# liznerski/eoe

Hardware: AMD Instinct MI355X
Metric: train images/sec, CLIP ViT-B/32 + HSC, 224x224 (higher is better)
Workload: dtype fp16; 1 GPU; CLIP ViT-B/32 (12 layers) + Linear(512,256) + HSC, full fine-tune, Adam lr 1e-4 wd 1e-3, 224x224, 128 normal + 128 OE images per GPU per step; global_batch=256, parallelism=dp1, launch=eager, weight-gradient launches on a side stream under the dgrad chain, arithmetic=16-bit MFMA operands, fp32 accumulate

## Files before the change

### eoe_amd/_lib.py

```python
import ctypes as C
import os
import re

import torch

from . import _build

ABI_VERSION = 5
EOE_F16, EOE_BF16, EOE_F32 = 1, 2, 3
EOE_RESIZE_BILINEAR, EOE_RESIZE_BICUBIC = 2, 3
EOE_MSM_LPF, EOE_MSM_HPF, EOE_MSM_BLUR = 1, 2, 3
EOE_MSM_FORM_NONE, EOE_MSM_FORM_DENSE, EOE_MSM_FORM_RANK = 0, 1, 2
EOE_GCN_L1, EOE_GCN_L2 = 1, 2
EOE_SALIENCY_MAX, EOE_SALIENCY_L2, EOE_SALIENCY_GRADXINPUT = 0, 1, 2
EOE_FUSE_MEAN, EOE_FUSE_MAX, EOE_FUSE_MIN = 0, 1, 2
EOE_CAM_GRADCAM, EOE_CAM_HIRESCAM = 0, 1
EOE_COMM_I64, EOE_COMM_ID_BYTES, EOE_COMM_ALGO_RING, EOE_COMM_ALGO_RS_AG = 8, 128, 0, 1
EPI_NONE, EPI_GELU, EPI_RESIDUAL, EPI_GELU_BWD = 0, 1, 2, 3
NT_KERNELS = ("none", "persistent_256x128", "persistent_256x96", "narrow_256x64", "persistent_narrow", "two_wg_128", "two_wg_160",
              "wide_160x256x32", "one_wave_160x256", "one_wave_256x256", "eight_wave", "eight_wave_stream_k", "split_k", "gather")
(NT_KERNEL_NONE, NT_KERNEL_PERSISTENT_256x128, NT_KERNEL_PERSISTENT_256x96, NT_KERNEL_NARROW_256x64, NT_KERNEL_PERSISTENT_NARROW,
 NT_KERNEL_TWO_WG_128, NT_KERNEL_TWO_WG_160, NT_KERNEL_WIDE_160x256x32, NT_KERNEL_ONE_WAVE_160x256, NT_KERNEL_ONE_WAVE_256x256,
 NT_KERNEL_EIGHT_WAVE, NT_KERNEL_EIGHT_WAVE_STREAM_K, NT_KERNEL_SPLIT_K, NT_KERNEL_GATHER) = range(14)
ADAM_CHUNK, ADAM_GROUPS = 8192, 4
# ... 100 lines not shown


class VitBlockBwdArgs(C.Structure):
    _fields_ = [("f", VitBlockFwdArgs), ("dx_out", _vp), ("dx_in", _vp),
                ("g_ln1_g", _vp), ("g_ln1_b", _vp), ("g_ln2_g", _vp), ("g_ln2_b", _vp),
                ("g_b_in", _vp), ("g_b_out", _vp), ("g_b_fc", _vp), ("g_b_proj", _vp),
                ("g_w_in", _vp), ("g_w_out", _vp), ("g_w_fc", _vp), ("g_w_proj", _vp),
                ("accumulate", _i32),
                ("d16_a", _vp), ("d16_b", _vp), ("d16_c", _vp), ("dh", _vp), ("dqkv", _vp), ("dx_mid", _vp), ("red_scratch", _vp),
                ("tn_workspace", _vp), ("tn_workspace_bytes", _i64),
                ("next_d16", _vp), ("in_d16", _vp), ("in_red_scratch", _vp), ("async_wgrad", _i32), ("red_table", C.POINTER(RedTable))]


ALLREDUCE_FN = C.CFUNCTYPE(C.c_int, C.c_void_p, C.c_void_p, C.c_int64, C.c_int, C.c_void_p)

SIGNATURES = {
    "eoe_abi_version": [],
    "eoe_struct_size": [C.c_int],
    "eoe_last_error": [],
    "eoe_vit_side_join": [_vp],
    "eoe_red_table_flush": [C.POINTER(RedTable), _vp],
    "eoe_gemm_nt": [C.POINTER(GemmArgs), _vp],
    "eoe_gemm_nt_route": [C.POINTER(GemmArgs), C.c_int, C.POINTER(C.c_int)],
    "eoe_gemm_tn": [C.POINTER(GemmArgs), _vp],
    "eoe_gemm_tn_grouped": [C.POINTER(GemmArgs), C.c_int, _vp],
    "eoe_cast_transpose": [_vp, _vp, _vp, C.c_int, C.c_int, C.c_int, _vp],
    "eoe_cast_transpose_multi": [_vp, C.c_int, C.c_int, _vp],
    "eoe_conv_pack_weight_multi": [_vp, C.c_int, C.c_int, _vp],
    "eoe_patchify": [_vp, _vp, _vp, _vp, C.c_int, C.c_int, C.c_int, C.c_int, _vp],
    "eoe_embed_lnpre_fwd": [_vp] * 8 + [C.c_int, C.c_int, C.c_int, _f32, _vp],
    "eoe_embed_lnpre_bwd": [_vp] * 10 + [C.c_int, C.c_int, C.c_int, C.c_int, _vp],
    "eoe_layernorm_fwd": [_vp, C.c_int, _vp, _vp, _vp, _vp, C.c_int, C.c_int, _f32, C.c_int, C.c_int, _vp],
    "eoe_layernorm_bwd": [_vp, C.c_int, _vp, C.c_int, _vp, _vp, _vp, _vp, C.c_int, _vp, _vp, _vp, _vp, _vp, C.c_int,
                          C.c_int, C.c_int, _vp],
    "eoe_linear_small_fwd": [_vp, _vp, _vp, _vp, C.c_int, C.c_int, C.c_int, _vp],
    "eoe_linear_small_bwd": [_vp, _vp, _vp, _vp, _vp, _vp, C.c_int, C.c_int, C.c_int, C.c_int, _vp],
    "eoe_zero_multi": [C.POINTER(_vp), C.POINTER(C.c_int), C.c_int, _vp],
    "eoe_cast_colsum": [_vp, _vp, _vp, _vp, C.c_int, C.c_int, C.c_int, C.c_int, _vp],
    "eoe_colsum": [_vp, C.c_int, _vp, C.c_int, C.c_int, C.c_int, C.c_int, _vp],
    "eoe_colsum_det": [_vp, C.c_int, _vp, _vp, C.c_int, C.c_int, C.c_int, _vp],
    "eoe_cast": [_vp, _vp, _sz, C.c_int, _vp],
    "eoe_attn_fwd": [_vp, _vp, C.c_int, C.c_int, C.c_int, C.c_int, _vp],
    "eoe_attn_bwd": [_vp, _vp, _vp, _vp, _vp, C.c_int, C.c_int, C.c_int, C.c_int, _vp],
    "eoe_attn_long_fwd": [_vp, _vp, C.c_int, C.c_int, C.c_int, C.c_int, _vp],
    "eoe_attn_long_bwd": [_vp, _vp, _vp, _vp, _vp, C.c_int, C.c_int, C.c_int, C.c_int, _vp],
    "eoe_attn_causal_fwd": [_vp, _vp, C.c_int, C.c_int, C.c_int, C.c_int, _vp],
# ... 167 lines not shown
            raise ImportError(f"eoe_amd: {cls.__name__} is {C.sizeof(cls)} bytes here but {lib.eoe_struct_size(idx)} in libeoe_hip.so "
                              "(the ctypes mirror and include/eoe_hip.h disagree)")
    return lib


def get_option(name: str) -> int:
    v = C.c_int(0)
    check(lib.eoe_get_option(name.encode(), C.byref(v)), "eoe_get_option")
    return v.value


def set_option(name: str, value: int) -> int:
    old = get_option(name)
    check(lib.eoe_set_option(name.encode(), int(value)), "eoe_set_option")
    return old


def gemm_nt_route(args: GemmArgs, ncu: int = 0) -> int:
    v = C.c_int(0)
    check(lib.eoe_gemm_nt_route(C.byref(args), int(ncu), C.byref(v)), "eoe_gemm_nt_route")
    return v.value


lib = _load()


class EoeError(RuntimeError):
    pass


def check(rc: int, what: str = ""):
    if rc != 0:
        msg = lib.eoe_last_error()
        raise EoeError(f"{what}: error {rc}: {msg.decode() if msg else ''}")


def prof_enable(on: bool):
    check(lib.eoe_prof_enable(1 if on else 0), "eoe_prof_enable")


def prof_collect():
    buf = (ProfEntry * 64)()
    n = C.c_int(0)
    check(lib.eoe_prof_collect(buf, 64, C.byref(n)), "eoe_prof_collect")
    return {buf[i].name.decode(): dict(launches=buf[i].launches, total_ms=buf[i].total_ms, flops=buf[i].flops,
                                       bytes=buf[i].bytes) for i in range(n.value)}
# ... 4 lines not shown
```

### eoe_amd/csrc/gemm.hip

```cpp
#include "gemm_common.h"
#include <stdlib.h>

unsigned long long* g_stamp_buf = nullptr;
extern int g_tn_flags;
extern int g_vit_side_stream;
extern int g_attn_flags;
extern int g_tn256_launches;
int g_nt_last_kernel = EOE_NT_KERNEL_NONE;
int g_nt_last_form = 0;
extern int g_parity_flags;
template <typename T> int eoe_launch_nt256(const void* gemm_p, int epi, int mi, hipStream_t s);
bool eoe_w8_applies(const void* gemm_p, int epi);
int eoe_w8_sk_rounds(const void* gemm_p, int flags, int ncu);
template <typename T> int eoe_launch_w8(const void* gemm_p, int epi, int sk_rounds, hipStream_t s);

namespace {


template <typename T, int EPI, int NI, int FLAGS, int GATHER = 0>
__global__ __launch_bounds__(512, 2) void gemm_nt_kernel(GemmP p) {
    extern __shared__ __attribute__((aligned(16))) char smem[];
    const int tid = threadIdx.x, lane = tid & 63, wave = tid >> 6;
    constexpr int BNI = 32 * NI;
    const int tiles_n = (p.N + BNI - 1) / BNI;
    const int total_tiles = tiles_n * ((p.M + BM - 1) / BM);
    const int G = gridDim.x;
    const int my_tiles = (total_tiles - (int)blockIdx.x + G - 1) / G;
    const int nk = p.K / BK;
// ... 732 lines not shown
    int split_s = 0;
    int sk_rounds = -1;
};

int nt128_rows_mi(const GemmP& p, int ncu, bool tie_to_160) {
    const int slots = 2 * ncu;
    const long t4 = (long)cdiv(p.M, 128) * cdiv(p.N, 128), t5 = (long)cdiv(p.M, 160) * cdiv(p.N, 128);
    const long c4 = (t4 + slots - 1) / slots * 128, c5 = (t5 + slots - 1) / slots * 160;
    return (c5 < c4 || (tie_to_160 && c5 == c4)) ? 5 : 4;
}

int nt_split_s(const GemmP& p, int epi, int flags, int ncu) {
    const int nk = p.K / BK;
    if ((flags & 8192) || !p.split_k || p.M > 1024 || nk < 24 || (epi != EOE_EPI_NONE && epi != EOE_EPI_RESIDUAL) || p.colsum || p.colsum_sq || p.accumulate ||
        (p.N & 15) || (p.ldc & 3) || (epi == EOE_EPI_RESIDUAL && (p.ldaux & 3)))
        return 0;
    int S = 8;
    while (S > 1 && (nk % S) != 0) S >>= 1;
    if (S < 2 || nk / S < 3) return 0;
    if (!p.sk_part || (size_t)S * p.M * p.N > (size_t)2 * ncu * 65536) return 0;
    return S;
}

NtRoute nt_route(const GemmP& p, int epi, int gather, int flags, int ncu) {
    if (epi == EOE_EPI_NONE && p.N <= 64 && (gather == 0 || gather == 1 || gather == 2) && !(flags & 64)) {
        return {gather ? EOE_NT_KERNEL_GATHER : EOE_NT_KERNEL_NARROW_256x64};
    }
    if (gather == 1 && epi == EOE_EPI_NONE && p.N >= 128 && !(flags & 2048)) {
        return {EOE_NT_KERNEL_GATHER, p.colsum_sq ? 4 : nt128_rows_mi(p, ncu, false)};
    }
    if (gather || (epi == EOE_EPI_NONE && p.N <= 64))
        return {gather ? EOE_NT_KERNEL_GATHER : EOE_NT_KERNEL_PERSISTENT_NARROW, 0, p.N <= 64 ? 2 : 4};
    if ((flags & (128 | 256)) && epilogue_direct_ok(p, epi))
        return (flags & 256) ? NtRoute{EOE_NT_KERNEL_ONE_WAVE_256x256, 8} : NtRoute{EOE_NT_KERNEL_ONE_WAVE_160x256, 5};
    const bool big = p.K >= 4096 && p.N >= 2048;
    if (const int S = nt_split_s(p, epi, flags, ncu)) return {EOE_NT_KERNEL_SPLIT_K, 4, 0, S};
    if (!(flags & (131072 | 4 | 8 | 512)) && p.M >= 2048 && eoe_w8_applies(&p, epi)) {
        const long tiles = (long)cdiv(p.M, 256) * (p.N / 256);
        const int sk_rounds = eoe_w8_sk_rounds(&p, flags, ncu);
        if (sk_rounds >= 0) return {EOE_NT_KERNEL_EIGHT_WAVE_STREAM_K, 0, 0, 0, sk_rounds};
        if ((flags & 262144) || tiles * 100 >= ((tiles + ncu - 1) / ncu) * ncu * 85) return {EOE_NT_KERNEL_EIGHT_WAVE};
    }
    if (!(flags & (4096 | 4 | 8 | 512)) && !p.colsum_sq && (p.N % 256) == 0 && p.N >= 2048 && (p.K % 32) == 0 && p.M >= 2048) {
        const long tiles = (long)cdiv(p.M, 160) * (p.N / 256), slots = 2L * ncu;
        if (tiles * 10 >= ((tiles + slots - 1) / slots) * slots * 9) return {EOE_NT_KERNEL_WIDE_160x256x32};
    }
    const bool gelu_wide = epi == EOE_EPI_GELU && p.N >= 2048 && p.K <= 1024 && !(flags & 1024);
    if (((flags & 512) || gelu_wide) && !(flags & (4 | 8)) && epilogue_direct_ok(p, epi) && p.M >= 2048 && p.N >= 512) {
        const int nk = p.K / BK;
        long best = 0;
        int mi_best = 5;
        for (int mi : {5, 8}) {
            const long tiles = (long)cdiv(p.M, 32 * mi) * cdiv(p.N, 256);
            const long cost = ((tiles + ncu - 1) / ncu) * ((long)mi * (nk + 2) + 30);
            if (!best || cost < best) { best = cost; mi_best = mi; }
        }
        return {mi_best == 8 ? EOE_NT_KERNEL_ONE_WAVE_256x256 : EOE_NT_KERNEL_ONE_WAVE_160x256, mi_best};
    }
    if (big && !(flags & (4 | 8)) && epilogue_direct_ok(p, epi) && p.M >= 2048) return {EOE_NT_KERNEL_ONE_WAVE_256x256, 8};
    if (!p.colsum_sq && ((flags & 8) || (!big && !(flags & 4)))) {
        const bool five = (flags & 32) || (!(flags & 16) && nt128_rows_mi(p, ncu, true) == 5);
        return five ? NtRoute{EOE_NT_KERNEL_TWO_WG_160, 5} : NtRoute{EOE_NT_KERNEL_TWO_WG_128, 4};
    }
    const int t4 = cdiv(p.M, BM) * cdiv(p.N, 128), t3 = cdiv(p.M, BM) * cdiv(p.N, 96);
    const int c4 = cdiv(t4, ncu) * 4, c3 = cdiv(t3, ncu) * 3;
    const int force = (flags >> 4) & 7;
    const bool use3 = force ? (force == 3) : (c3 * 10 <= c4 * 9);
    return use3 ? NtRoute{EOE_NT_KERNEL_PERSISTENT_256x96, 0, 3} : NtRoute{EOE_NT_KERNEL_PERSISTENT_256x128, 0, 4};
}

template <typename T>
int launch_nt(const GemmP& p, int epi, int gather, hipStream_t s) {
    const int flags = g_nt_flags, ncu = num_cus();
    const NtRoute r = nt_route(p, epi, gather, flags, ncu);
    g_nt_last_kernel = r.kernel;
    g_nt_last_form = r.mi * 16 + r.ni;
    switch (r.kernel) {
        case EOE_NT_KERNEL_NARROW_256x64:
        case EOE_NT_KERNEL_GATHER:
            if (!r.mi && !r.ni) return gather == 2 ? launch_nt64<T, 2>(p, s) : (gather ? launch_nt64<T, 1>(p, s) : launch_nt64<T, 0>(p, s));
            if (r.mi) return r.mi == 5 ? launch_nt128_gather<T, 5>(p, s) : launch_nt128_gather<T, 4>(p, s);
            if (gather == 2) return r.ni == 2 ? launch_nt_conv<T, 2, 2>(p, ncu, s) : launch_nt_conv<T, 4, 2>(p, ncu, s);
            if (gather == 3) return r.ni == 2 ? launch_nt_conv<T, 2, 3>(p, ncu, s) : launch_nt_conv<T, 4, 3>(p, ncu, s);
            return r.ni == 2 ? launch_nt_conv<T, 2, 1>(p, ncu, s) : launch_nt_conv<T, 4, 1>(p, ncu, s);
        case EOE_NT_KERNEL_PERSISTENT_NARROW: return launch_nt_conv<T, 2, 0>(p, ncu, s);
        case EOE_NT_KERNEL_ONE_WAVE_160x256:
        case EOE_NT_KERNEL_ONE_WAVE_256x256: return eoe_launch_nt256<T>(&p, epi, r.mi, s);
        case EOE_NT_KERNEL_SPLIT_K: return launch_nt128_splitk<T>(p, epi, r.split_s, s);
        case EOE_NT_KERNEL_EIGHT_WAVE:
        case EOE_NT_KERNEL_EIGHT_WAVE_STREAM_K: return eoe_launch_w8<T>(&p, epi, r.sk_rounds, s);
        case EOE_NT_KERNEL_WIDE_160x256x32: return launch_nt128w<T>(p, epi, s);
        case EOE_NT_KERNEL_TWO_WG_160: return launch_nt128<T, 5>(p, epi, s);
        case EOE_NT_KERNEL_TWO_WG_128: return launch_nt128<T, 4>(p, epi, s);
        case EOE_NT_KERNEL_PERSISTENT_256x96: return launch_nt_ni<T, 3>(p, epi, flags, ncu, s);
        default: return launch_nt_ni<T, 4>(p, epi, flags, ncu, s);
    }
}
// ... 67 lines not shown
        EOE_CHECK_ARG(a->workspace && a->workspace_bytes >= 2 * (int64_t)EOE_NT_COLSUM_WORKSPACE_BYTES(a->M, a->N),
                      "gemm_nt: colstats needs a workspace of 2 * EOE_NT_COLSUM_WORKSPACE_BYTES(M, N)");
        EOE_CHECK_ARG((a->N & 15) == 0 && (a->ldc & 7) == 0 && (a->ldaux & 7) == 0 && (((uintptr_t)a->C) & 15) == 0,
                      "gemm_nt: colstats needs N %% 16 == 0 and 16-byte aligned rows of C");
        p.colsum_part = (float*)a->workspace;
        p.colsum_sq = 1;
        p.colsum_blocked = 0;
    }
    return 0;
}

void attach_stamps(GemmP& p) {
    static const int stampon = getenv("EOE_GEMM_STAMP") ? atoi(getenv("EOE_GEMM_STAMP")) : 0;
    if (stampon) {
        static unsigned long long* buf = [] { void* b = nullptr; (void)hipMalloc(&b, 4096 * 16 * 8); return (unsigned long long*)b; }();
        (void)hipMemsetAsync(buf, 0, 4096 * 16 * 8, 0);
        p.stamp = buf;
        g_stamp_buf = buf;
    }
}

}

extern "C" int eoe_gemm_nt(const eoe_gemm_args* a, void* stream) {
    GemmP p;
    int mode;
    EOE_TRY(fill_params(a, num_cus(), p, mode));
    attach_stamps(p);
    const int osz = a->out_f32 ? 4 : 2;
    static const bool by_shape = getenv("EOE_PROF_SHAPES") != nullptr;
    char pname[32] = "gemm_nt";
    if (by_shape) snprintf(pname, sizeof(pname), "nt_%dx%dx%d_e%d%s", a->M, a->N, a->K, a->epilogue, a->colsum ? "c" : "");
    ProfScope ps(pname, 2.0 * a->M * a->N * a->K,
                 2.0 * ((a->gather ? (double)a->geo.n * a->geo.H * a->geo.W * a->geo.C : (double)a->M * a->K) + (double)a->N * a->K) +
                     (double)osz * a->M * a->N *
                     (a->epilogue == EOE_EPI_GELU ? 2 : 1) + (a->epilogue == EOE_EPI_RESIDUAL ? 4.0 * a->M * a->N : 0.0) +
                     (a->epilogue == EOE_EPI_GELU_BWD ? 2.0 * a->M * a->N : 0.0), stream);
    return a->dtype == EOE_F16 ? launch_nt<f16_t>(p, a->epilogue, mode, (hipStream_t)stream)
                               : launch_nt<bf16_t>(p, a->epilogue, mode, (hipStream_t)stream);
}

extern "C" int eoe_gemm_nt_route(const eoe_gemm_args* a, int ncu, int* kernel) {
    EOE_CHECK_ARG(kernel != nullptr, "eoe_gemm_nt_route: null pointer");
    if (ncu <= 0) ncu = num_cus();
    GemmP p;
    int mode;
    EOE_TRY(fill_params(a, ncu, p, mode));
    *kernel = nt_route(p, a->epilogue, mode, g_nt_flags, ncu).kernel;
    return 0;
}

extern "C" int eoe_debug_gemm_stamps(unsigned long long* out, int n_words) {
    if (!g_stamp_buf || !out) return eoe_set_error(EOE_ERR_ARG, "gemm stamps are not enabled (EOE_GEMM_STAMP=1)");
    if (hipDeviceSynchronize() != hipSuccess) return eoe_set_error(EOE_ERR_LAUNCH, "sync failed");
    if (hipMemcpy(out, g_stamp_buf, (size_t)n_words * 8, hipMemcpyDeviceToHost) != hipSuccess)
        return eoe_set_error(EOE_ERR_LAUNCH, "copy failed");
    return 0;
}

extern "C" int eoe_set_option(const char* name, int value) {
    if (name && !strcmp(name, "nt_flags")) { g_nt_flags = value; return 0; }
    if (name && !strcmp(name, "tn_flags")) { g_tn_flags = value; return 0; }
    if (name && !strcmp(name, "vit_side_stream")) { g_vit_side_stream = value; return 0; }
    if (name && !strcmp(name, "attn_flags")) { g_attn_flags = value; return 0; }
    if (name && !strcmp(name, "parity_flags")) { g_parity_flags = value; return 0; }
    return eoe_set_error(EOE_ERR_ARG, "unknown option");
}

extern "C" int eoe_get_option(const char* name, int* value) {
    EOE_CHECK_ARG(name && value, "eoe_get_option: null pointer");
    if (!strcmp(name, "nt_flags")) { *value = g_nt_flags; return 0; }
    if (!strcmp(name, "tn_flags")) { *value = g_tn_flags; return 0; }
    if (!strcmp(name, "vit_side_stream")) { *value = g_vit_side_stream; return 0; }
    if (!strcmp(name, "attn_flags")) { *value = g_attn_flags; return 0; }
    if (!strcmp(name, "tn256_launches")) { *value = g_tn256_launches; return 0; }
    if (!strcmp(name, "nt_last_kernel")) { *value = g_nt_last_kernel; return 0; }
    if (!strcmp(name, "nt_last_form")) { *value = g_nt_last_form; return 0; }
    if (!strcmp(name, "parity_flags")) { *value = g_parity_flags; return 0; }
    return eoe_set_error(EOE_ERR_ARG, "unknown option");
}
```

### eoe_amd/csrc/vit.cpp

```cpp
#include "common.h"
#include <mutex>
#include <stdlib.h>

#define TRY(expr)                   \
    do {                            \
        int rc__ = (expr);          \
        if (rc__ != 0) return rc__; \
    } while (0)

extern int g_tn_flags;
bool eoe_tn_streamk_would_run(const eoe_gemm_args* args, int count, void* stream);
int eoe_red_table_append(eoe_red_table* t, EoeRedJobs* jobs, void* stream);
int g_vit_side_stream = 1;

namespace {

struct SideStream {
    hipStream_t s = nullptr;
    hipEvent_t fork = nullptr, join = nullptr, wgrad_done[2] = {nullptr, nullptr};
    bool ok = false;
    unsigned seq = 0;
    bool recorded[2] = {false, false};
};
SideStream* side_stream(hipStream_t main) {
    static SideStream per_dev[16];
    static std::mutex mu;
    std::lock_guard<std::mutex> lk(mu);
    int dev = 0;
    if (hipGetDevice(&dev) != hipSuccess || dev < 0 || dev >= 16) return nullptr;
    SideStream& ss = per_dev[dev];
    hipStreamCaptureStatus st = hipStreamCaptureStatusNone;
    if (hipStreamIsCapturing(main, &st) != hipSuccess || st != hipStreamCaptureStatusNone) return nullptr;
    if (!ss.ok) {
        int lo = 0, hi = 0;
        (void)hipDeviceGetStreamPriorityRange(&lo, &hi);
        if (hipStreamCreateWithPriority(&ss.s, hipStreamNonBlocking, lo) != hipSuccess) return nullptr;
        if (hipEventCreateWithFlags(&ss.fork, hipEventDisableTiming) != hipSuccess ||
            hipEventCreateWithFlags(&ss.join, hipEventDisableTiming) != hipSuccess ||
            hipEventCreateWithFlags(&ss.wgrad_done[0], hipEventDisableTiming) != hipSuccess ||
            hipEventCreateWithFlags(&ss.wgrad_done[1], hipEventDisableTiming) != hipSuccess)
            return nullptr;
        ss.ok = true;
    }
    return &ss;
}

eoe_gemm_args gemm(const void* A, const void* B, void* C, const float* bias, int M, int N, int K, int lda, int ldb,
                   int ldc, int dtype) {
    eoe_gemm_args g = {};
    g.A = A; g.B = B; g.C = C; g.bias = bias; g.aux = nullptr; g.aux_out = nullptr; g.colsum = nullptr;
    g.M = M; g.N = N; g.K = K; g.lda = lda; g.ldb = ldb; g.ldc = ldc; g.ldaux = 0;
    g.dtype = dtype; g.epilogue = EOE_EPI_NONE; g.out_f32 = 0; g.accumulate = 0; g.alpha = 1.0f;
    return g;
}
eoe_gemm_args gemm(const eoe_vit_block_fwd_args* a, const void* A, const void* B, void* C, const float* bias, int M, int N, int K, int lda,
                   int ldb, int ldc, int dtype) {
    eoe_gemm_args g = gemm(A, B, C, bias, M, N, K, lda, ldb, ldc, dtype);
    g.sk_workspace = a->nt_sk_workspace; g.sk_workspace_bytes = a->nt_sk_workspace ? a->nt_sk_workspace_bytes : 0;
    return g;
}

int check_fwd(const eoe_vit_block_fwd_args* a) {
    if (!a) return eoe_set_error(EOE_ERR_ARG, "vit_block: null args");
    if (a->n <= 0 || a->L <= 0 || a->L > EOE_ATTN_LONG_MAX_L || a->heads <= 0 || a->D != a->heads * 64)
        return eoe_set_error(EOE_ERR_ARG, "vit_block: unsupported shape n=%d L=%d D=%d heads=%d (need D = 64*heads, L <= %d)",
                             a->n, a->L, a->D, a->heads, EOE_ATTN_LONG_MAX_L);
    if (!a->ln1_g || !a->ln1_b || !a->ln2_g || !a->ln2_b || !a->b_in || !a->b_out || !a->b_fc || !a->b_proj || !a->w_in ||
        !a->w_out || !a->w_fc || !a->w_proj || !a->x_in || !a->x_mid || !a->x_out || !a->xn1 || !a->qkv || !a->att ||
        !a->xn2 || !a->hact || !a->stats1 || !a->stats2)
        return eoe_set_error(EOE_ERR_ARG, "vit_block: null pointer in arguments");
    return 0;
}

}

extern "C" int eoe_vit_block_fwd(const eoe_vit_block_fwd_args* a, void* stream) {
    TRY(check_fwd(a));
    const int M = a->n * a->L, D = a->D, H = 4 * a->D, dt = a->dtype;
    TRY(eoe_layernorm_fwd(a->x_in, D, a->ln1_g, a->ln1_b, a->xn1, a->stats1, M, D, a->eps, dt, 0, stream));
    eoe_gemm_args g = gemm(a, a->xn1, a->w_in, a->qkv, a->b_in, M, 3 * D, D, D, D, 3 * D, dt);
    TRY(eoe_gemm_nt(&g, stream));
    TRY(a->L <= 64 ? eoe_attn_fwd(a->qkv, a->att, a->n, a->L, a->heads, dt, stream)
                   : eoe_attn_long_fwd(a->qkv, a->att, a->n, a->L, a->heads, dt, stream));
    const int Mo = a->cls_only ? a->n : M, ldrow = a->cls_only ? a->L * D : D;
    g = gemm(a, a->att, a->w_out, a->x_mid, a->b_out, Mo, D, D, ldrow, D, D, dt);
    g.epilogue = EOE_EPI_RESIDUAL; g.aux = a->x_in; g.ldaux = ldrow; g.out_f32 = 1;
    TRY(eoe_gemm_nt(&g, stream));
    TRY(eoe_layernorm_fwd(a->x_mid, D, a->ln2_g, a->ln2_b, a->xn2, a->stats2, Mo, D, a->eps, dt, 0, stream));
    g = gemm(a, a->xn2, a->w_fc, a->hact, a->b_fc, Mo, H, D, D, D, H, dt);
    g.epilogue = EOE_EPI_GELU; g.aux_out = a->hpre;
    TRY(eoe_gemm_nt(&g, stream));
    g = gemm(a, a->hact, a->w_proj, a->x_out, a->b_proj, Mo, D, H, H, H, D, dt);
    g.epilogue = EOE_EPI_RESIDUAL; g.aux = a->x_mid; g.ldaux = D; g.out_f32 = 1;
    g.split_k = a->cls_only ? 1 : 0;
    TRY(eoe_gemm_nt(&g, stream));
    return 0;
}

extern "C" int eoe_vit_block_bwd(const eoe_vit_block_bwd_args* b, void* stream) {
    if (!b) return eoe_set_error(EOE_ERR_ARG, "vit_block_bwd: null args");
    const eoe_vit_block_fwd_args* a = &b->f;
    TRY(check_fwd(a));
    if (!a->hpre || !a->w_in_t || !a->w_out_t || !a->w_fc_t || !a->w_proj_t || !b->dx_out || !b->dx_in || !b->g_ln1_g || !b->g_ln1_b ||
        !b->g_ln2_g || !b->g_ln2_b || !b->g_b_in || !b->g_b_out || !b->g_b_fc || !b->g_b_proj || !b->g_w_in || !b->g_w_out ||
        !b->g_w_fc || !b->g_w_proj || !b->d16_a || !b->d16_b || !b->d16_c || !b->dh || !b->dqkv || !b->dx_mid)
        return eoe_set_error(EOE_ERR_ARG, "vit_block_bwd: null pointer in arguments");
    const int M = a->n * a->L, D = a->D, H = 4 * a->D, dt = a->dtype, acc = b->accumulate;
    hipStream_t s = (hipStream_t)stream;
    const bool cls = a->cls_only != 0;
    const int Mo = cls ? a->n : M, ldrow = cls ? a->L * D : D;
    if (cls && a->L < 4) return eoe_set_error(EOE_ERR_ARG, "vit_block_bwd: cls_only needs L >= 4");
    if (!acc && !b->red_scratch) {
        float* zp[8] = {b->g_ln1_g, b->g_ln1_b, b->g_ln2_g, b->g_ln2_b, b->g_b_fc, b->g_b_out, b->g_b_proj, b->g_b_in};
        const int zn[8] = {D, D, D, D, H, D, D, 3 * D};
        TRY(eoe_zero_multi(zp, zn, 8, stream));
    }
    EoeRedJobs jobs;
    jobs.count = 0; jobs.tile_start[0] = 0; jobs.overwrite = acc ? 0 : 1;
    struct DeferGuard {
        explicit DeferGuard(EoeRedJobs* j) { eoe_tls_defer = j; }
        ~DeferGuard() { eoe_tls_defer = nullptr; }
    } guard(b->red_scratch ? &jobs : nullptr);
    float* red_fc = b->red_scratch;
    float* red_ln2 = red_fc ? red_fc + (size_t)((M + 63) / 64) * H : nullptr;
    float* red_attn = red_fc ? red_ln2 + EOE_LN_SCRATCH(D) : nullptr;
// ... 110 lines not shown
```

### eoe_amd/models/clip_vit.py

```python
import math
from collections import OrderedDict

import torch
from torch import nn

from .. import ops


def is_causal_mask(m) -> bool:
    if not isinstance(m, torch.Tensor) or m.dim() != 2 or m.shape[0] != m.shape[1] or not m.is_floating_point():
        return False
    want = torch.full(m.shape, float("-inf"), dtype=m.dtype, device=m.device).triu_(1)
    return bool(torch.equal(m, want))


class _PackedAttention(nn.Module):

    def __init__(self, d_model: int, n_head: int):
        super().__init__()
        self.embed_dim, self.num_heads = d_model, n_head
        self.in_proj_weight = nn.Parameter(torch.empty(3 * d_model, d_model))
        self.in_proj_bias = nn.Parameter(torch.empty(3 * d_model))
        self.out_proj = nn.Linear(d_model, d_model)
        self._reset_parameters()
# ... 81 lines not shown

    def set_normalize(self, mean, std):
        if mean is None:
            self.normalize = None
        else:
            dev = self.proj.device
            self.normalize = (torch.as_tensor(mean, dtype=torch.float32, device=dev).contiguous(),
                              torch.as_tensor(std, dtype=torch.float32, device=dev).contiguous())

    def embed(self, x: torch.Tensor) -> torch.Tensor:
        if not x.is_cuda:
            raise RuntimeError("eoe_amd.VisualTransformer runs on the GPU only (no CPU fallback)")
        mean, std = self.normalize if self.normalize is not None else (None, None)
        ops.shadow.refresh([w for blk in self.transformer.resblocks
                            for w in (blk.attn.in_proj_weight, blk.attn.out_proj.weight, blk.mlp.c_fc.weight, blk.mlp.c_proj.weight)]
                           + [self.proj])
        return ops.VitEmbedFunction.apply(x, self.conv1.weight, self.class_embedding, self.positional_embedding,
                                          self.ln_pre.weight, self.ln_pre.bias, self.patch_size, mean, std)

    def forward(self, x: torch.Tensor) -> torch.Tensor:
        n = x.shape[0]
        tok = self.embed(x)
        blocks = list(self.transformer.resblocks)
        for i, blk in enumerate(blocks):
            tok = blk.forward_tokens(tok, n, cls_only=ops.VIT_CLS_ONLY_LAST and i == len(blocks) - 1)
        return ops.VitHeadFunction.apply(tok, n, self.ln_post.weight, self.ln_post.bias, self.proj)


def convert_weights(model: nn.Module) -> nn.Module:
    def mark(p):
        if p is None:
            return
        with torch.no_grad():
            p.copy_(p.to(torch.float16).to(torch.float32))
        p._eoe_fp16_weight = True

    for m in model.modules():
        if isinstance(m, (nn.Conv1d, nn.Conv2d, nn.Linear)):
            mark(m.weight)
            mark(m.bias)
        if isinstance(m, (_PackedAttention, nn.MultiheadAttention)):
            for name in ("in_proj_weight", "q_proj_weight", "k_proj_weight", "v_proj_weight", "in_proj_bias", "bias_k", "bias_v"):
                mark(getattr(m, name, None))
        for name in ("text_projection", "proj"):
            attr = getattr(m, name, None)
            if isinstance(attr, nn.Parameter):
                mark(attr)
    return model
# ... 1 lines not shown
```

### eoe_amd/ops.py

```python
import ctypes as C
import math
import os
import weakref
from collections import namedtuple
from typing import NamedTuple, Optional

import torch

from . import _lib
from ._lib import lib, check, GemmArgs, EPI_NONE, EPI_GELU, EPI_RESIDUAL, EPI_GELU_BWD

_compute_dtype = torch.float16


def set_compute_dtype(dt):
    global _compute_dtype
    if isinstance(dt, str):
        dt = {"bf16": torch.bfloat16, "bfloat16": torch.bfloat16, "fp16": torch.float16, "f16": torch.float16,
              "float16": torch.float16}[dt]
    if dt not in (torch.bfloat16, torch.float16):
        raise ValueError(f"unsupported compute dtype {dt}")
    _compute_dtype = dt


# ... 486 lines not shown
        self.seq = 0
        if self.table.count:
            check(lib.eoe_red_table_flush(C.byref(self.table), self.stream), "eoe_red_table_flush")


_vit_sweeps = {}


def _vit_live_sweeps():
    task = torch._C._current_graph_task_id()
    return [sw for sw in _vit_sweeps.values() if sw.task == task]


def vit_flush_finish():
    for sw in _vit_live_sweeps():
        sw.flush()


def vit_side_join():
    vit_flush_finish()
    check(lib.eoe_vit_side_join(_stream()), "eoe_vit_side_join")
    for sw in _vit_live_sweeps():
        sw.pending = None


VIT_CLS_ONLY_LAST = os.environ.get("EOE_VIT_CLS_ONLY", "1") != "0"


class VitBlockFunction(torch.autograd.Function):

    @staticmethod
    def forward(ctx, x, n, heads, ln1_g, ln1_b, w_in, b_in, w_out, b_out, ln2_g, ln2_b, w_fc, b_fc, w_proj, b_proj, cls_only=False):
        _chk(x)
        x = x.contiguous()
        M, D = x.shape
        L = M // n
        ws, ptr = _block_ws(M, D, x.device, _compute_dtype)
        cls_only = bool(cls_only) and L >= 4
        x_out = x.new_empty((n, D)) if cls_only else torch.empty_like(x)
        need_t = torch.is_grad_enabled()
        sh = {k: shadow.get(w, True, True) for k, w in (("in", w_in), ("out", w_out), ("fc", w_fc), ("proj", w_proj))}
        sk_ws = nt_sk_workspace(x.device)
        code = dtype_code(_compute_dtype)
        sig = (n, L, D, heads, code, _p(ln1_g), _p(ln1_b), _p(ln2_g), _p(ln2_b), _p(b_in), _p(b_out), _p(b_fc), _p(b_proj),
               _p(sh["in"][0]), _p(sh["out"][0]), _p(sh["fc"][0]), _p(sh["proj"][0]), _p(sh["in"][1]), _p(sh["out"][1]), _p(sh["fc"][1]),
               _p(sh["proj"][1]), _p(sk_ws))
# ... 2 lines not shown
            a = _lib.VitBlockFwdArgs.from_buffer_copy(hit[1])
        else:
            a = _lib.VitBlockFwdArgs()
            a.n, a.L, a.D, a.heads, a.dtype, a.eps = n, L, D, heads, code, 1e-5
            a.ln1_g, a.ln1_b, a.ln2_g, a.ln2_b = _p(ln1_g), _p(ln1_b), _p(ln2_g), _p(ln2_b)
            a.b_in, a.b_out, a.b_fc, a.b_proj = _p(b_in), _p(b_out), _p(b_fc), _p(b_proj)
            a.w_in, a.w_out, a.w_fc, a.w_proj = (_p(sh[k][0]) for k in ("in", "out", "fc", "proj"))
            a.w_in_t, a.w_out_t, a.w_fc_t, a.w_proj_t = (_p(sh[k][1]) for k in ("in", "out", "fc", "proj"))
            a.nt_sk_workspace, a.nt_sk_workspace_bytes = _p(sk_ws), sk_ws.numel()
            if len(_vit_args_cache) > 256:
                _vit_args_cache.clear()
            _vit_args_cache[id(w_in)] = (sig, bytes(a))
        a.x_in, a.x_mid, a.x_out = _p(x), ptr["x_mid"], _p(x_out)
        a.xn1, a.qkv, a.att, a.xn2, a.hpre, a.hact = (ptr[k] for k in ("xn1", "qkv", "att", "xn2", "hpre", "hact"))
        a.stats1, a.stats2 = ptr["stats1"], ptr["stats2"]
        a.cls_only = 1 if cls_only else 0
        sw = _vit_sweeps.get((x.device.index, _stream()))
        if sw is not None and sw.table.count and sw.task != torch._C._current_graph_task_id():
            sw.table.count = 0
        keep = any(ctx.needs_input_grad)
        if not keep:
            a.hpre = None
        check(lib.eoe_vit_block_fwd(C.byref(a), _stream()), "eoe_vit_block_fwd")
        ctx.save_for_backward(x, ws, ln1_g, ln1_b, w_in, b_in, w_out, b_out, ln2_g, ln2_b, w_fc, b_fc, w_proj, b_proj)
        ctx.args = a
        ctx.shadows = sh
        ctx.sk_ws = sk_ws
        return x_out

    @staticmethod
    def backward(ctx, dx_out):
        saved = ctx.saved_tensors
        x, ws = saved[0], saved[1]
        params = dict(zip(_BLOCK_PARAMS, saved[2:]))
        M, D = x.shape
        dev = x.device
        dt = torch.float16 if ctx.args.dtype == _lib.EOE_F16 else torch.bfloat16
        dx_out = dx_out.contiguous()
        dx_in = torch.empty_like(x)
        grads = {k: _grad_target(p) for k, p in params.items()}
        b = _lib.VitBlockBwdArgs()
        b.f = ctx.args
        b.dx_out, b.dx_in = _p(dx_out), _p(dx_in)
        b.g_ln1_g, b.g_ln1_b, b.g_ln2_g, b.g_ln2_b = (_p(grads[k]) for k in ("ln1_g", "ln1_b", "ln2_g", "ln2_b"))
        b.g_b_in, b.g_b_out, b.g_b_fc, b.g_b_proj = (_p(grads[k]) for k in ("b_in", "b_out", "b_fc", "b_proj"))
        b.g_w_in, b.g_w_out, b.g_w_fc, b.g_w_proj = (_p(grads[k]) for k in ("w_in", "w_out", "w_fc", "w_proj"))
# ... 1030 lines not shown
```

### include/eoe_hip.h

```cpp
#ifndef EOE_HIP_H
#define EOE_HIP_H

#include <stddef.h>
#include <stdint.h>

#ifdef __cplusplus
extern "C" {
#endif

#define EOE_ABI_VERSION 5

enum { EOE_OK = 0, EOE_ERR_ARG = 1, EOE_ERR_LAUNCH = 2, EOE_ERR_UNSUPPORTED = 3 };
enum { EOE_F16 = 1, EOE_BF16 = 2, EOE_F32 = 3  };

int eoe_abi_version(void);
int eoe_struct_size(int which);
const char* eoe_last_error(void);

enum {
    EOE_EPI_NONE = 0,
    EOE_EPI_GELU = 1,
    EOE_EPI_RESIDUAL = 2,
    EOE_EPI_GELU_BWD = 3
};
// ... 201 lines not shown
    float *g_w_in, *g_w_out, *g_w_fc, *g_w_proj;
    int32_t accumulate;
    void *d16_a;
    void *d16_b;
    void *d16_c;
    void *dh;
    void *dqkv;
    float* dx_mid;
    float* red_scratch;
    void* tn_workspace;
    int64_t tn_workspace_bytes;
    void* next_d16;
    const void* in_d16;
    const float* in_red_scratch;
    int32_t async_wgrad;
    struct eoe_red_table* red_table;
} eoe_vit_block_bwd_args;

#define EOE_VIT_RED_SCRATCH(n, L, D) \
    ((size_t)(((size_t)(n) * (L) + 63) / 64) * 4 * (D) + 2 * EOE_LN_SCRATCH(D) + (size_t)(n) * 3 * (D) + (size_t)EOE_CAST_COLSUM_PARTIALS * (D))
int eoe_vit_block_fwd(const eoe_vit_block_fwd_args* a, void* stream);
int eoe_vit_block_bwd(const eoe_vit_block_bwd_args* a, void* stream);
int eoe_vit_side_join(void* stream);

int eoe_im2col(const void* x, int x_kind, const float* mean, const float* std, void* out, int n, int cin, int H, int W,
               int kh, int kw, int stride, int pad, int Kp, int dtype, void* stream);
int eoe_col2im(const void* dpatches, float* dx, int n, int C, int H, int W, int kh, int kw, int stride, int pad, int Kp,
               int dtype, int accumulate , void* stream);
typedef struct {
    const float* w;
    void *w16, *w16t, *w16d;
    int32_t cout, cin, cpad, kh, kw, Kp;
} eoe_conv_pack_job;
int eoe_conv_pack_weight_multi(const eoe_conv_pack_job* jobs, int count, int dtype, void* stream);
int eoe_conv_pack_weight(const float* w, void* w16, void* w16t, void* w16d, int cout, int cin, int cpad, int kh, int kw,
                         int Kp, int dtype, void* stream);
int eoe_conv_unpack_wgrad(const float* g, float* dw, int cout, int cin, int cpad, int kh, int kw, int Kp, int transposed,
                          int accumulate, void* stream);
int eoe_stem_pack_image(const float* x, const float* mean, const float* std, void* out, int n, int H, int W, int Hp, int Wp,
                        int pad, int cpad ,
                        int dtype, void* stream);
int eoe_stem_pack_weight(const float* w, void* w16, int cout, int kh, int kw, int dtype, void* stream);
int eoe_stem_unpack_wgrad(const float* g, float* dw, int cout, int kh, int kw, void* stream);

#define EOE_BN_PARTIALS 1024
#define EOE_BN_SCRATCH(C) ((EOE_BN_PARTIALS + 3) * 2 * (C))
// ... 264 lines not shown

int eoe_probe_mfma_f16(float* out, int iters, int blocks, void* stream);
int eoe_probe_copy(void* dst, const void* src, int64_t bytes, void* stream);

int eoe_set_option(const char* name, int value);
int eoe_get_option(const char* name, int* value);
enum {
    EOE_NT_KERNEL_NONE = 0,
    EOE_NT_KERNEL_PERSISTENT_256x128 = 1,
    EOE_NT_KERNEL_PERSISTENT_256x96 = 2,
    EOE_NT_KERNEL_NARROW_256x64 = 3,
    EOE_NT_KERNEL_PERSISTENT_NARROW = 4,
    EOE_NT_KERNEL_TWO_WG_128 = 5,
    EOE_NT_KERNEL_TWO_WG_160 = 6,
    EOE_NT_KERNEL_WIDE_160x256x32 = 7,
    EOE_NT_KERNEL_ONE_WAVE_160x256 = 8,
    EOE_NT_KERNEL_ONE_WAVE_256x256 = 9,
    EOE_NT_KERNEL_EIGHT_WAVE = 10,
    EOE_NT_KERNEL_EIGHT_WAVE_STREAM_K = 11,
    EOE_NT_KERNEL_SPLIT_K = 12,
    EOE_NT_KERNEL_GATHER = 13
};
int eoe_gemm_nt_route(const eoe_gemm_args* args, int ncu, int* kernel);
int eoe_debug_gemm_stamps(unsigned long long* out, int n_words);
int eoe_prof_collect(eoe_prof_entry* out, int max_entries, int* n_out);

#ifdef __cplusplus
}
#endif
#endif
```

Measured before the change: 25890 images/sec.

## Split ViT forward into two image-band chains on main and side streams

The ViT block forward now splits the batch into two halves of images. Each half runs its own layernorm/GEMM/attention chain, one on the main stream and one on the side stream, so the two chains can overlap across all blocks until a join before the CLS-only last block or before the backward. GEMM routing for each half is chosen as if for the full row count, with stream-K disabled, so the smaller GEMMs keep the full-size kernel choice. The aim is to fill idle CUs and hide per-kernel serialization and tail effects. The cost is extra event synchronization and lifetime bookkeeping (held tensors), plus possible contention from smaller per-half GEMMs.

```diff
diff --git a/eoe_amd/_lib.py b/eoe_amd/_lib.py
--- a/eoe_amd/_lib.py
+++ b/eoe_amd/_lib.py
@@ -146,6 +146,9 @@
     "eoe_red_table_flush": [C.POINTER(RedTable), _vp],
     "eoe_gemm_nt": [C.POINTER(GemmArgs), _vp],
     "eoe_gemm_nt_route": [C.POINTER(GemmArgs), C.c_int, C.POINTER(C.c_int)],
+    "eoe_gemm_nt_band_route": [C.POINTER(GemmArgs), C.c_int, C.c_int, C.POINTER(C.c_int), C.POINTER(C.c_int)],
+    "eoe_vit_fwd_fork": [_vp],
+    "eoe_vit_fwd_join": [_vp],
     "eoe_gemm_tn": [C.POINTER(GemmArgs), _vp],
     "eoe_gemm_tn_grouped": [C.POINTER(GemmArgs), C.c_int, _vp],
     "eoe_cast_transpose": [_vp, _vp, _vp, C.c_int, C.c_int, C.c_int, _vp],
@@ -359,6 +362,12 @@
     return v.value
 
 
+def gemm_nt_band_route(args: GemmArgs, route_m: int, ncu: int = 0):
+    v, f = C.c_int(0), C.c_int(0)
+    check(lib.eoe_gemm_nt_band_route(C.byref(args), int(route_m), int(ncu), C.byref(v), C.byref(f)), "eoe_gemm_nt_band_route")
+    return v.value, f.value
+
+
 lib = _load()
 
 
diff --git a/eoe_amd/csrc/gemm.hip b/eoe_amd/csrc/gemm.hip
--- a/eoe_amd/csrc/gemm.hip
+++ b/eoe_amd/csrc/gemm.hip
@@ -4,6 +4,8 @@
 unsigned long long* g_stamp_buf = nullptr;
 extern int g_tn_flags;
 extern int g_vit_side_stream;
+extern int g_vit_fwd_chains;
+int eoe_vit_fwd_forked();
 extern int g_attn_flags;
 extern int g_tn256_launches;
 int g_nt_last_kernel = EOE_NT_KERNEL_NONE;
@@ -782,7 +784,7 @@
     return S;
 }
 
-NtRoute nt_route(const GemmP& p, int epi, int gather, int flags, int ncu) {
+NtRoute nt_route_rows(const GemmP& p, int epi, int gather, int flags, int ncu) {
     if (epi == EOE_EPI_NONE && p.N <= 64 && (gather == 0 || gather == 1 || gather == 2) && !(flags & 64)) {
         return {gather ? EOE_NT_KERNEL_GATHER : EOE_NT_KERNEL_NARROW_256x64};
     }
@@ -829,10 +831,23 @@
     return use3 ? NtRoute{EOE_NT_KERNEL_PERSISTENT_256x96, 0, 3} : NtRoute{EOE_NT_KERNEL_PERSISTENT_256x128, 0, 4};
 }
 
+NtRoute nt_route(const GemmP& p, int epi, int gather, int flags, int ncu, int route_m = 0) {
+    if (route_m <= p.M) return nt_route_rows(p, epi, gather, flags, ncu);
+    GemmP q = p;
+    q.M = route_m;
+    NtRoute r = nt_route_rows(q, epi, gather, flags, ncu);
+    if (r.kernel == EOE_NT_KERNEL_EIGHT_WAVE || r.kernel == EOE_NT_KERNEL_EIGHT_WAVE_STREAM_K) {
+        if (!eoe_w8_applies(&p, epi)) return nt_route_rows(p, epi, gather, flags, ncu);
+        r.kernel = EOE_NT_KERNEL_EIGHT_WAVE;
+        r.sk_rounds = -1;
+    }
+    return r;
+}
+
 template <typename T>
-int launch_nt(const GemmP& p, int epi, int gather, hipStream_t s) {
+int launch_nt(const GemmP& p, int epi, int gather, int route_m, hipStream_t s) {
     const int flags = g_nt_flags, ncu = num_cus();
-    const NtRoute r = nt_route(p, epi, gather, flags, ncu);
+    const NtRoute r = nt_route(p, epi, gather, flags, ncu, route_m);
     g_nt_last_kernel = r.kernel;
     g_nt_last_form = r.mi * 16 + r.ni;
     switch (r.kernel) {
@@ -946,7 +961,7 @@
 
 }
 
-extern "C" int eoe_gemm_nt(const eoe_gemm_args* a, void* stream) {
+int eoe_gemm_nt_band(const eoe_gemm_args* a, int route_m, void* stream) {
     GemmP p;
     int mode;
     EOE_TRY(fill_params(a, num_cus(), p, mode));
@@ -960,17 +975,23 @@
                      (double)osz * a->M * a->N *
                      (a->epilogue == EOE_EPI_GELU ? 2 : 1) + (a->epilogue == EOE_EPI_RESIDUAL ? 4.0 * a->M * a->N : 0.0) +
                      (a->epilogue == EOE_EPI_GELU_BWD ? 2.0 * a->M * a->N : 0.0), stream);
-    return a->dtype == EOE_F16 ? launch_nt<f16_t>(p, a->epilogue, mode, (hipStream_t)stream)
-                               : launch_nt<bf16_t>(p, a->epilogue, mode, (hipStream_t)stream);
-}
-
-extern "C" int eoe_gemm_nt_route(const eoe_gemm_args* a, int ncu, int* kernel) {
+    return a->dtype == EOE_F16 ? launch_nt<f16_t>(p, a->epilogue, mode, route_m, (hipStream_t)stream)
+                               : launch_nt<bf16_t>(p, a->epilogue, mode, route_m, (hipStream_t)stream);
+}
+
+extern "C" int eoe_gemm_nt(const eoe_gemm_args* a, void* stream) { return eoe_gemm_nt_band(a, 0, stream); }
+
+extern "C" int eoe_gemm_nt_route(const eoe_gemm_args* a, int ncu, int* kernel) { return eoe_gemm_nt_band_route(a, 0, ncu, kernel, nullptr); }
+
+extern "C" int eoe_gemm_nt_band_route(const eoe_gemm_args* a, int route_m, int ncu, int* kernel, int* form) {
     EOE_CHECK_ARG(kernel != nullptr, "eoe_gemm_nt_route: null pointer");
     if (ncu <= 0) ncu = num_cus();
     GemmP p;
     int mode;
     EOE_TRY(fill_params(a, ncu, p, mode));
-    *kernel = nt_route(p, a->epilogue, mode, g_nt_flags, ncu).kernel;
+    const NtRoute r = nt_route(p, a->epilogue, mode, g_nt_flags, ncu, route_m);
+    *kernel = r.kernel;
+    if (form) *form = r.mi * 16 + r.ni + 256 * r.split_s;
     return 0;
 }
 
@@ -986,6 +1007,7 @@
     if (name && !strcmp(name, "nt_flags")) { g_nt_flags = value; return 0; }
     if (name && !strcmp(name, "tn_flags")) { g_tn_flags = value; return 0; }
     if (name && !strcmp(name, "vit_side_stream")) { g_vit_side_stream = value; return 0; }
+    if (name && !strcmp(name, "vit_fwd_chains")) { g_vit_fwd_chains = value; return 0; }
     if (name && !strcmp(name, "attn_flags")) { g_attn_flags = value; return 0; }
     if (name && !strcmp(name, "parity_flags")) { g_parity_flags = value; return 0; }
     return eoe_set_error(EOE_ERR_ARG, "unknown option");
@@ -996,6 +1018,8 @@
     if (!strcmp(name, "nt_flags")) { *value = g_nt_flags; return 0; }
     if (!strcmp(name, "tn_flags")) { *value = g_tn_flags; return 0; }
     if (!strcmp(name, "vit_side_stream")) { *value = g_vit_side_stream; return 0; }
+    if (!strcmp(name, "vit_fwd_chains")) { *value = g_vit_fwd_chains; return 0; }
+    if (!strcmp(name, "vit_fwd_forked")) { *value = eoe_vit_fwd_forked(); return 0; }
     if (!strcmp(name, "attn_flags")) { *value = g_attn_flags; return 0; }
     if (!strcmp(name, "tn256_launches")) { *value = g_tn256_launches; return 0; }
     if (!strcmp(name, "nt_last_kernel")) { *value = g_nt_last_kernel; return 0; }
diff --git a/eoe_amd/csrc/vit.cpp b/eoe_amd/csrc/vit.cpp
--- a/eoe_amd/csrc/vit.cpp
+++ b/eoe_amd/csrc/vit.cpp
@@ -11,7 +11,9 @@
 extern int g_tn_flags;
 bool eoe_tn_streamk_would_run(const eoe_gemm_args* args, int count, void* stream);
 int eoe_red_table_append(eoe_red_table* t, EoeRedJobs* jobs, void* stream);
+int eoe_gemm_nt_band(const eoe_gemm_args* a, int route_m, void* stream);
 int g_vit_side_stream = 1;
+int g_vit_fwd_chains = 2;
 
 namespace {
 
@@ -21,11 +23,20 @@
     bool ok = false;
     unsigned seq = 0;
     bool recorded[2] = {false, false};
+    hipEvent_t fwd_fork = nullptr, fwd_join = nullptr;
+    hipStream_t fwd_main = nullptr;
+    bool fwd_forked = false;
 };
+SideStream per_dev[16];
+std::mutex per_dev_mu;
+SideStream* forked_on(hipStream_t main) {
+    int dev = 0;
+    if (hipGetDevice(&dev) != hipSuccess || dev < 0 || dev >= 16) return nullptr;
+    SideStream& ss = per_dev[dev];
+    return ss.ok && ss.fwd_forked && ss.fwd_main == main ? &ss : nullptr;
+}
 SideStream* side_stream(hipStream_t main) {
-    static SideStream per_dev[16];
-    static std::mutex mu;
-    std::lock_guard<std::mutex> lk(mu);
+    std::lock_guard<std::mutex> lk(per_dev_mu);
     int dev = 0;
     if (hipGetDevice(&dev) != hipSuccess || dev < 0 || dev >= 16) return nullptr;
     SideStream& ss = per_dev[dev];
@@ -38,7 +49,9 @@
         if (hipEventCreateWithFlags(&ss.fork, hipEventDisableTiming) != hipSuccess ||
             hipEventCreateWithFlags(&ss.join, hipEventDisableTiming) != hipSuccess ||
             hipEventCreateWithFlags(&ss.wgrad_done[0], hipEventDisableTiming) != hipSuccess ||
-            hipEventCreateWithFlags(&ss.wgrad_done[1], hipEventDisableTiming) != hipSuccess)
+            hipEventCreateWithFlags(&ss.wgrad_done[1], hipEventDisableTiming) != hipSuccess ||
+            hipEventCreateWithFlags(&ss.fwd_fork, hipEventDisableTiming) != hipSuccess ||
+            hipEventCreateWithFlags(&ss.fwd_join, hipEventDisableTiming) != hipSuccess)
             return nullptr;
         ss.ok = true;
     }
@@ -72,35 +85,98 @@
     return 0;
 }
 
-}
-
-extern "C" int eoe_vit_block_fwd(const eoe_vit_block_fwd_args* a, void* stream) {
-    TRY(check_fwd(a));
+int fwd_chain(const eoe_vit_block_fwd_args* a, int route_m, void* stream) {
     const int M = a->n * a->L, D = a->D, H = 4 * a->D, dt = a->dtype;
     TRY(eoe_layernorm_fwd(a->x_in, D, a->ln1_g, a->ln1_b, a->xn1, a->stats1, M, D, a->eps, dt, 0, stream));
     eoe_gemm_args g = gemm(a, a->xn1, a->w_in, a->qkv, a->b_in, M, 3 * D, D, D, D, 3 * D, dt);
-    TRY(eoe_gemm_nt(&g, stream));
+    TRY(eoe_gemm_nt_band(&g, route_m, stream));
     TRY(a->L <= 64 ? eoe_attn_fwd(a->qkv, a->att, a->n, a->L, a->heads, dt, stream)
                    : eoe_attn_long_fwd(a->qkv, a->att, a->n, a->L, a->heads, dt, stream));
     const int Mo = a->cls_only ? a->n : M, ldrow = a->cls_only ? a->L * D : D;
     g = gemm(a, a->att, a->w_out, a->x_mid, a->b_out, Mo, D, D, ldrow, D, D, dt);
     g.epilogue = EOE_EPI_RESIDUAL; g.aux = a->x_in; g.ldaux = ldrow; g.out_f32 = 1;
-    TRY(eoe_gemm_nt(&g, stream));
+    TRY(eoe_gemm_nt_band(&g, route_m, stream));
     TRY(eoe_layernorm_fwd(a->x_mid, D, a->ln2_g, a->ln2_b, a->xn2, a->stats2, Mo, D, a->eps, dt, 0, stream));
     g = gemm(a, a->xn2, a->w_fc, a->hact, a->b_fc, Mo, H, D, D, D, H, dt);
     g.epilogue = EOE_EPI_GELU; g.aux_out = a->hpre;
-    TRY(eoe_gemm_nt(&g, stream));
+    TRY(eoe_gemm_nt_band(&g, route_m, stream));
     g = gemm(a, a->hact, a->w_proj, a->x_out, a->b_proj, Mo, D, H, H, H, D, dt);
     g.epilogue = EOE_EPI_RESIDUAL; g.aux = a->x_mid; g.ldaux = D; g.out_f32 = 1;
     g.split_k = a->cls_only ? 1 : 0;
-    TRY(eoe_gemm_nt(&g, stream));
-    return 0;
+    TRY(eoe_gemm_nt_band(&g, route_m, stream));
+    return 0;
+}
+
+eoe_vit_block_fwd_args image_band(const eoe_vit_block_fwd_args* a, int n0, int n1) {
+    eoe_vit_block_fwd_args b = *a;
+    const size_t r0 = (size_t)n0 * a->L, D = (size_t)a->D;
+    b.n = n1 - n0;
+    b.x_in = a->x_in + r0 * D; b.x_mid = a->x_mid + r0 * D; b.x_out = a->x_out + r0 * D;
+    b.xn1 = (char*)a->xn1 + r0 * D * 2; b.qkv = (char*)a->qkv + r0 * 3 * D * 2; b.att = (char*)a->att + r0 * D * 2;
+    b.xn2 = (char*)a->xn2 + r0 * D * 2; b.hact = (char*)a->hact + r0 * 4 * D * 2;
+    b.hpre = a->hpre ? (char*)a->hpre + r0 * 4 * D * 2 : nullptr;
+    b.stats1 = a->stats1 + r0 * 2; b.stats2 = a->stats2 + r0 * 2;
+    b.nt_sk_workspace = nullptr; b.nt_sk_workspace_bytes = 0;
+    return b;
+}
+
+int fwd_join(SideStream* ss, hipStream_t s) {
+    ss->fwd_forked = false;
+    ss->fwd_main = nullptr;
+    if (hipEventRecord(ss->fwd_join, ss->s) != hipSuccess || hipStreamWaitEvent(s, ss->fwd_join, 0) != hipSuccess)
+        return eoe_set_error(EOE_ERR_LAUNCH, "vit_fwd_join: join failed");
+    return 0;
+}
+
+}
+
+extern "C" int eoe_vit_block_fwd(const eoe_vit_block_fwd_args* a, void* stream) {
+    TRY(check_fwd(a));
+    hipStream_t s = (hipStream_t)stream;
+    if (SideStream* ss = forked_on(s)) {
+        hipStreamCaptureStatus st = hipStreamCaptureStatusNone;
+        if (hipStreamIsCapturing(s, &st) != hipSuccess || st != hipStreamCaptureStatusNone)
+            return eoe_set_error(EOE_ERR_ARG, "vit_block: stream capture between eoe_vit_fwd_fork and eoe_vit_fwd_join");
+        if (a->n >= 2 && !a->cls_only && g_vit_fwd_chains >= 2 && g_vit_side_stream) {
+            const int n_a = (a->n + 1) / 2, M = a->n * a->L;
+            const eoe_vit_block_fwd_args lo = image_band(a, 0, n_a), hi = image_band(a, n_a, a->n);
+            TRY(fwd_chain(&lo, M, stream));
+            return fwd_chain(&hi, M, (void*)ss->s);
+        }
+        TRY(fwd_join(ss, s));
+    }
+    return fwd_chain(a, 0, stream);
+}
+
+int eoe_vit_fwd_forked() {
+    int dev = 0;
+    return hipGetDevice(&dev) == hipSuccess && dev >= 0 && dev < 16 && per_dev[dev].ok && per_dev[dev].fwd_forked ? 1 : 0;
+}
+
+extern "C" int eoe_vit_fwd_fork(void* stream) {
+    hipStream_t s = (hipStream_t)stream;
+    if (g_vit_fwd_chains < 2 || !g_vit_side_stream) return 0;
+    SideStream* ss = side_stream(s);
+    if (!ss) return 0;
+    if (ss->fwd_forked) return eoe_set_error(EOE_ERR_ARG, "vit_fwd_fork: the forward of this device is forked already (eoe_vit_fwd_join first)");
+    if (hipEventRecord(ss->fwd_fork, s) != hipSuccess || hipStreamWaitEvent(ss->s, ss->fwd_fork, 0) != hipSuccess)
+        return eoe_set_error(EOE_ERR_LAUNCH, "vit_fwd_fork: fork failed");
+    ss->fwd_forked = true;
+    ss->fwd_main = s;
+    return 0;
+}
+
+extern "C" int eoe_vit_fwd_join(void* stream) {
+    hipStream_t s = (hipStream_t)stream;
+    SideStream* ss = forked_on(s);
+    return ss ? fwd_join(ss, s) : 0;
 }
 
 extern "C" int eoe_vit_block_bwd(const eoe_vit_block_bwd_args* b, void* stream) {
     if (!b) return eoe_set_error(EOE_ERR_ARG, "vit_block_bwd: null args");
     const eoe_vit_block_fwd_args* a = &b->f;
     TRY(check_fwd(a));
+    if (SideStream* fs = forked_on((hipStream_t)stream)) TRY(fwd_join(fs, (hipStream_t)stream));
     if (!a->hpre || !a->w_in_t || !a->w_out_t || !a->w_fc_t || !a->w_proj_t || !b->dx_out || !b->dx_in || !b->g_ln1_g || !b->g_ln1_b ||
         !b->g_ln2_g || !b->g_ln2_b || !b->g_b_in || !b->g_b_out || !b->g_b_fc || !b->g_b_proj || !b->g_w_in || !b->g_w_out ||
         !b->g_w_fc || !b->g_w_proj || !b->d16_a || !b->d16_b || !b->d16_c || !b->dh || !b->dqkv || !b->dx_mid)
diff --git a/eoe_amd/models/clip_vit.py b/eoe_amd/models/clip_vit.py
--- a/eoe_amd/models/clip_vit.py
+++ b/eoe_amd/models/clip_vit.py
@@ -127,8 +127,17 @@
         n = x.shape[0]
         tok = self.embed(x)
         blocks = list(self.transformer.resblocks)
-        for i, blk in enumerate(blocks):
-            tok = blk.forward_tokens(tok, n, cls_only=ops.VIT_CLS_ONLY_LAST and i == len(blocks) - 1)
+        last_cls = ops.VIT_CLS_ONLY_LAST and len(blocks) > 0
+        forked = n >= 2 and len(blocks) > int(last_cls) and ops.vit_fwd_fork()
+        try:
+            for i, blk in enumerate(blocks):
+                if forked and last_cls and i == len(blocks) - 1:
+                    ops.vit_fwd_join()
+                    forked = False
+                tok = blk.forward_tokens(tok, n, cls_only=last_cls and i == len(blocks) - 1)
+        finally:
+            if forked:
+                ops.vit_fwd_join()
         return ops.VitHeadFunction.apply(tok, n, self.ln_post.weight, self.ln_post.bias, self.proj)
 
 
diff --git a/eoe_amd/ops.py b/eoe_amd/ops.py
--- a/eoe_amd/ops.py
+++ b/eoe_amd/ops.py
@@ -532,6 +532,26 @@
     check(lib.eoe_vit_side_join(_stream()), "eoe_vit_side_join")
     for sw in _vit_live_sweeps():
         sw.pending = None
+
+
+_vit_fwd_held = []
+_vit_fwd_forked = False
+
+
+def vit_fwd_fork():
+    global _vit_fwd_forked
+    check(lib.eoe_vit_fwd_fork(_stream()), "eoe_vit_fwd_fork")
+    _vit_fwd_forked = _lib.get_option("vit_fwd_forked") == 1
+    return _vit_fwd_forked
+
+
+def vit_fwd_join():
+    global _vit_fwd_forked
+    try:
+        check(lib.eoe_vit_fwd_join(_stream()), "eoe_vit_fwd_join")
+    finally:
+        _vit_fwd_forked = False
+        _vit_fwd_held.clear()
 
 
 VIT_CLS_ONLY_LAST = os.environ.get("EOE_VIT_CLS_ONLY", "1") != "0"
@@ -580,6 +600,8 @@
         if not keep:
             a.hpre = None
         check(lib.eoe_vit_block_fwd(C.byref(a), _stream()), "eoe_vit_block_fwd")
+        if _vit_fwd_forked:
+            _vit_fwd_held.append((x, ws, x_out))
         ctx.save_for_backward(x, ws, ln1_g, ln1_b, w_in, b_in, w_out, b_out, ln2_g, ln2_b, w_fc, b_fc, w_proj, b_proj)
         ctx.args = a
         ctx.shadows = sh
diff --git a/include/eoe_hip.h b/include/eoe_hip.h
--- a/include/eoe_hip.h
+++ b/include/eoe_hip.h
@@ -247,6 +247,8 @@
 int eoe_vit_block_fwd(const eoe_vit_block_fwd_args* a, void* stream);
 int eoe_vit_block_bwd(const eoe_vit_block_bwd_args* a, void* stream);
 int eoe_vit_side_join(void* stream);
+int eoe_vit_fwd_fork(void* stream);
+int eoe_vit_fwd_join(void* stream);
 
 int eoe_im2col(const void* x, int x_kind, const float* mean, const float* std, void* out, int n, int cin, int H, int W,
                int kh, int kw, int stride, int pad, int Kp, int dtype, void* stream);
@@ -557,6 +559,7 @@
     EOE_NT_KERNEL_GATHER = 13
 };
 int eoe_gemm_nt_route(const eoe_gemm_args* args, int ncu, int* kernel);
+int eoe_gemm_nt_band_route(const eoe_gemm_args* args, int route_m, int ncu, int* kernel, int* form);
 int eoe_debug_gemm_stamps(unsigned long long* out, int n_words);
 int eoe_prof_collect(eoe_prof_entry* out, int max_entries, int* n_out);
 
```

Result: no change. 26080 images/sec, median of 6 (+0.7%).
